# stm233/image-compression-for-machine

Measured on AMD Instinct MI355X. Metric: images/sec (256x256) cnn-hyperprior (WACNN) training step, higher is better.
Workload: dtype f32; 1 GPU; cnn (WACNN N=192 M=320) train step, lambda=0.0067 MSE, batch 16/GPU synthetic 256x256, Adam lr 1e-4 + aux Adam, clip 1.0; global_batch=16, parallelism=dp1

## Files before the change

image-compression-for-machine_amd/csrc/conv_igemm.hip:

```cpp
#include <cstdlib>
#include <vector>
#include "conv_common.h"

namespace icm {

template <int WCO, int WPX, int TCO, int TPX, int KS = 1>
__global__ __launch_bounds__(512, (TCO * TPX <= 3) ? 4 : 2) void conv_igemm_kernel(const ConvDesc d) {
  extern __shared__ __attribute__((aligned(16))) float smem[];
  static_assert(WCO * WPX * KS == 4, "4 MFMA waves per workgroup");
  constexpr int BCO_T = WCO * TCO;
  constexpr int TS = (TCO * TPX == 1) ? 3 : ((TCO * TPX == 2) ? 2 : 1);
  const int tid = threadIdx.x, lane = tid & 63, wave = tid >> 6;
  const bool loader = wave >= 4;
  const ConvPtrs P = d.g[blockIdx.y];
  const PatchGeom& pg = d.pg;

  int bid = xcd_block_id();
  const int cb = bid % d.ncb;
  int pt = bid / d.ncb;
  const int tx_i = pt % d.tiles_x;
  pt /= d.tiles_x;
  const int ty_i = pt % d.tiles_y;
  const int tn_i = pt / d.tiles_y;
  const int ox0 = tx_i << d.lgTW, oy0 = ty_i << d.lgTH, n0 = tn_i << d.lgTI;
  const int S_in = pg.S == 2 ? 2 : 1;
  const int iyb = oy0 * S_in + d.iy0, ixb = ox0 * S_in + d.ix0;
  const int bufsz = d.ckm * 8 * pg.CS;
  const int nchunks = (d.nchunks8 + d.ckm - 1) / d.ckm;

  if (loader) {
    const int lw = __builtin_amdgcn_readfirstlane(wave) - 4;
    PlaneMap pm;

    if (pg.dma) {
      plane_map_init(pm, pg, n0, iyb, ixb, lane);
      stage_planes_dma(P.x, pm, pg, 0, min(d.ckm, d.nchunks8) * 8, smem, lw, lane);
      asm volatile("s_waitcnt vmcnt(0)" ::: "memory");
      __syncthreads();
      for (int chunk = 0; chunk < nchunks; ++chunk) {
        if (chunk + 1 < nchunks) {
          const int c8 = (chunk + 1) * d.ckm;
          stage_planes_dma(P.x, pm, pg, c8 * 8, min(d.ckm, d.nchunks8 - c8) * 8, smem + ((chunk + 1) & 1) * bufsz, lw, lane);
          asm volatile("s_waitcnt vmcnt(0)" ::: "memory");
        }
        __syncthreads();
      }
      return;
    }
    if (pg.vec4) {
      plane_map_init_v4(pm, pg, n0, iyb, ixb, lane);
      stage_planes_v4<8>(P.x, pm, pg, 0, min(d.ckm, d.nchunks8) * 8, smem, lw);
      __syncthreads();
      for (int chunk = 0; chunk < nchunks; ++chunk) {
        if (chunk + 1 < nchunks) {
          const int c8 = (chunk + 1) * d.ckm;
          stage_planes_v4<8>(P.x, pm, pg, c8 * 8, min(d.ckm, d.nchunks8 - c8) * 8, smem + ((chunk + 1) & 1) * bufsz,
                             lw);
        }
        __syncthreads();
      }
      return;
    }
    plane_map_init(pm, pg, n0, iyb, ixb, lane);
    stage_planes<12>(P.x, pm, pg, 0, min(d.ckm, d.nchunks8) * 8, smem, lw);
    __syncthreads();
    for (int chunk = 0; chunk < nchunks; ++chunk) {
      if (chunk + 1 < nchunks) {
        const int c8 = (chunk + 1) * d.ckm;
        stage_planes<12>(P.x, pm, pg, c8 * 8, min(d.ckm, d.nchunks8 - c8) * 8, smem + ((chunk + 1) & 1) * bufsz, lw);
      }
      __syncthreads();
    }
    return;
  }

  const int wave_u = __builtin_amdgcn_readfirstlane(wave);
  const int wk = wave_u % KS, wsp = wave_u / KS;
  const int wco = wsp / WPX, wpx = wsp % WPX;
  const int h = lane >> 5, l31 = lane & 31;
  const int TWm = (1 << d.lgTW) - 1, THm = (1 << d.lgTH) - 1;
  const int rowmul = S_in * pg.PWrow;
  int boff[TPX];
// ... 57 lines not shown
        const int qq = (st * TS + u) * KS + wk;
        const int qc = min(qq, nq - 1);
        ok_n[u] = (qq < nq) ? 1.0f : 0.0f;
        const float* bp = cur + __builtin_amdgcn_readlane(step_lane, qc);
#pragma unroll
        for (int j = 0; j < 4; ++j)
#pragma unroll
          for (int tp = 0; tp < TPX; ++tp) bv_n[u][j][tp] = bp[boff[tp] + 2 * j * pg.CS];
      };
      auto half_step = [&](f32x4 (&aq)[TS][TCO], int st) {
        float bv[TS][4][TPX];
#pragma unroll
        for (int u = 0; u < TS; ++u)
#pragma unroll
          for (int j = 0; j < 4; ++j)
#pragma unroll
            for (int tp = 0; tp < TPX; ++tp) bv[u][j][tp] = bv_n[u][j][tp] * ok_n[u];
        const int stn = min(st + 1, nsteps2 - 1);
#pragma unroll
        for (int u = 0; u < TS; ++u) {
          const char* sp = wptr(chunk, st + 2, u);
#pragma unroll
          for (int a = 0; a < TCO; ++a) {
#pragma unroll
            for (int tp = 0; tp < TPX; ++tp)
#pragma unroll
              for (int j = 0; j < 4; ++j)
                acc[a][tp] = __builtin_amdgcn_mfma_f32_32x32x2f32(aq[u][a][j], bv[u][j][tp], acc[a][tp], 0, 0, 0);
            if (a == 0) bload(stn, u);
            aq[u][a] = *reinterpret_cast<const f32x4*>(sp + wl[a]);
            __builtin_amdgcn_sched_barrier(0);
          }
        }
      };
#pragma unroll
      for (int u = 0; u < TS; ++u) bload(0, u);
      for (int st = 0; st < nsteps2; st += 2) {
        half_step(aq0, st);
        half_step(aq1, st + 1);
      }
      __syncthreads();
    }
  }

  if constexpr (KS > 1) {
    static_assert(TCO == 1 && TPX == 1, "split-K configurations hold one tile per wave");
    float* red = smem + (wsp * (KS - 1)) * 1024;
    if (wk > 0) {
#pragma unroll
      for (int r = 0; r < 16; ++r) red[(wk - 1) * 1024 + r * 64 + lane] = acc[0][0][r];
    }
    __syncthreads();
    if (wk > 0) return;
#pragma unroll
    for (int k = 0; k < KS - 1; ++k)
#pragma unroll
      for (int r = 0; r < 16; ++r) acc[0][0][r] += red[k * 1024 + r * 64 + lane];
  }
  {
    int pn[TPX], poy[TPX], pox[TPX];
    bool pv[TPX];
#pragma unroll
    for (int tp = 0; tp < TPX; ++tp) {
      const int p = (wpx * TPX + tp) * 32 + l31;
      const int tx = p & TWm, ty = (p >> d.lgTW) & THm, ti = p >> (d.lgTW + d.lgTH);
      const int oyv = oy0 + ty, oxv = ox0 + tx;
      pn[tp] = n0 + ti;
      pv[tp] = (pn[tp] < d.pg.N) && (oyv < d.OHv) && (oxv < d.OWv);
      poy[tp] = oyv * d.out_sy + d.out_oy;
      pox[tp] = oxv * d.out_sx + d.out_ox;
    }
    epilogue_dispatch<TCO, TPX>(d, P, acc, cot0, h, pn, poy, pox, pv);
  }
}

struct PackDesc {
  const float* w;
  float* wp;
  int Co, Ci, KHW, src_out_major, ntaps, ncot, nchunks, nonneg;
  float bound, pedestal;
  int src_ld, src_off;
  int dst_ncot, dst_cot_off;
  int wino;
  short tapidx[ICM_MAX_TAPS];
};

#define ICM_PACK_LDS (8 * 32 * ICM_MAX_TAPS + 64)
__device__ __forceinline__ void pack_unit(const PackDesc& d, int cot, int chunk, float* lds) {
  const int KHW = d.KHW, tid = threadIdx.x;
  const int co0 = cot * 32, ci0 = chunk * 8;
  int rows, rlen, rstride;
  if (d.src_out_major) { rows = 32; rlen = 8 * KHW; } else { rows = 8; rlen = 32 * KHW; }
  rstride = rlen | 1;
  const int total = rows * rlen;
  for (int e0 = tid; e0 < total; e0 += 8 * (int)blockDim.x) {
    float v[8];
    int lo[8];
#pragma unroll
    for (int u = 0; u < 8; ++u) {
      const int e = e0 + u * (int)blockDim.x;
      v[u] = 0.0f;
      lo[u] = -1;
      if (e < total) {
        const int r = e / rlen, c = e - r * rlen;
        lo[u] = r * rstride + c;
        if (d.src_out_major) {
          const int co = co0 + r, ci = ci0 + c / KHW;
          if (co < d.Co && ci < d.Ci) v[u] = d.w[((long long)co * d.src_ld + d.src_off + ci0) * KHW + c];
        } else {
          const int ci = ci0 + r, co = co0 + c / KHW;
          if (ci < d.Ci && co < d.Co) v[u] = d.w[((long long)ci * d.src_ld + d.src_off + co0) * KHW + c];
        }
      }
    }
#pragma unroll
    for (int u = 0; u < 8; ++u) {
      if (lo[u] >= 0) {
        float x = v[u];
        if (d.nonneg) {
          x = fmaxf(x, d.bound);
          x = x * x - d.pedestal;
        }
        lds[lo[u]] = x;
      }
    }
  }
  __syncthreads();
  f32x4* out = reinterpret_cast<f32x4*>(d.wp);
  for (int e = tid; e < d.ntaps * 64; e += blockDim.x) {
    const int t = e >> 6, lane = e & 63;
    const int col = lane & 31, hh = lane >> 5, k = d.tapidx[t];
    f32x4 o;
#pragma unroll
    for (int j = 0; j < 4; ++j) {
      const int cil = 2 * j + hh;
      const float* gsrc = d.src_out_major ? lds + col * rstride + cil * KHW : lds + cil * rstride + col * KHW;
      float v;
      if (d.wino) {
        const int wa = t >> 2, wb = t & 3;
        float row[3];
#pragma unroll
        for (int p = 0; p < 3; ++p) {
          const float g0 = gsrc[d.wino == 2 ? (2 - p) * 3 + 2 : p * 3 + 0];
          const float g1 = gsrc[d.wino == 2 ? (2 - p) * 3 + 1 : p * 3 + 1];
          const float g2 = gsrc[d.wino == 2 ? (2 - p) * 3 + 0 : p * 3 + 2];
          row[p] = wb == 0 ? g0 : (wb == 3 ? g2 : (wb == 1 ? 0.5f * ((g0 + g2) + g1) : 0.5f * ((g0 + g2) - g1)));
        }
        v = wa == 0 ? row[0] : (wa == 3 ? row[2] : (wa == 1 ? 0.5f * ((row[0] + row[2]) + row[1]) : 0.5f * ((row[0] + row[2]) - row[1])));
      } else {
        v = gsrc[k];
      }
      const bool valid = (co0 + col < d.Co) && (ci0 + cil < d.Ci);
      o[j] = valid ? v : 0.0f;
    }
    out[((long long)(chunk * d.ntaps + t) * d.dst_ncot + d.dst_cot_off + cot) * 64 + lane] = o;
  }
  __syncthreads();
}

__global__ __launch_bounds__(256) void pack_weights_kernel(const PackDesc d) {
  __shared__ float lds[ICM_PACK_LDS];
  const int units = d.ncot * d.nchunks;
  for (int u = blockIdx.x; u < units; u += gridDim.x) pack_unit(d, u % d.ncot, u / d.ncot, lds);
}

#define ICM_PACK_NB 24
struct PackMulti {
  PackDesc g[ICM_PACK_NB];
};
__global__ __launch_bounds__(256) void pack_weights_multi_kernel(const PackMulti m) {
  __shared__ float lds[ICM_PACK_LDS];
  const PackDesc& d = m.g[blockIdx.y];
  const int units = d.ncot * d.nchunks;
  for (int u = blockIdx.x; u < units; u += gridDim.x) pack_unit(d, u % d.ncot, u / d.ncot, lds);
}

struct Tap {
  int kidx;
  int dy, dx;
};
struct ConvClass {
  int cy, cx;
  int iy0, ix0;
  int ey, ex;
  std::vector<Tap> taps;
};

static void axis_taps(int K, int s, int pad, int c, std::vector<int>& ks, std::vector<int>& dis) {
  for (int k = 0; k < K; ++k) {
    const int v = c + pad - k;
    if (((v % s) + s) % s != 0) continue;
    ks.push_back(k);
    dis.push_back(v >= 0 ? v / s : -((-v) / s));
  }
}

static std::vector<ConvClass> build_classes(int KH, int KW, int stride, int pad, int transposed) {
  std::vector<ConvClass> out;
  if (!transposed) {
    ConvClass c;
    c.cy = c.cx = 0;
    c.iy0 = c.ix0 = -pad;
    c.ey = KH;
    c.ex = KW;
    for (int kh = 0; kh < KH; ++kh)
      for (int kw = 0; kw < KW; ++kw) c.taps.push_back({kh * KW + kw, kh, kw});
    out.push_back(c);
    return out;
  }
  for (int cy = 0; cy < stride; ++cy)
    for (int cx = 0; cx < stride; ++cx) {
      std::vector<int> khs, dys, kws, dxs;
      axis_taps(KH, stride, pad, cy, khs, dys);
      axis_taps(KW, stride, pad, cx, kws, dxs);
      ConvClass c;
      c.cy = cy;
      c.cx = cx;
      int miny = 0, minx = 0, maxy = 0, maxx = 0;
      for (size_t i = 0; i < dys.size(); ++i) {
        miny = i ? std::min(miny, dys[i]) : dys[i];
        maxy = i ? std::max(maxy, dys[i]) : dys[i];
      }
      for (size_t i = 0; i < dxs.size(); ++i) {
        minx = i ? std::min(minx, dxs[i]) : dxs[i];
        maxx = i ? std::max(maxx, dxs[i]) : dxs[i];
      }
      c.iy0 = miny;
      c.ix0 = minx;
      c.ey = maxy - miny + 1;
      c.ex = maxx - minx + 1;
      for (size_t a = 0; a < khs.size(); ++a)
        for (size_t b = 0; b < kws.size(); ++b)
          c.taps.push_back({khs[a] * KW + kws[b], dys[a] - miny, dxs[b] - minx});
      out.push_back(c);
    }
  return out;
}

struct KernelCfg {
  int wco, wpx, tco, tpx;
  void (*fn)(const ConvDesc);
  int ks;
  double eff;
  int occ;
};
static const KernelCfg kCfgs[] = {
    {1, 4, 3, 2, conv_igemm_kernel<1, 4, 3, 2>, 1, 0.75, 1},
    {1, 4, 6, 1, conv_igemm_kernel<1, 4, 6, 1>, 1, 1.00, 1},
    {1, 4, 2, 2, conv_igemm_kernel<1, 4, 2, 2>, 1, 0.80, 1},
    {1, 4, 1, 2, conv_igemm_kernel<1, 4, 1, 2>, 1, 0.60, 2},
    {1, 4, 3, 1, conv_igemm_kernel<1, 4, 3, 1>, 1, 1.10, 2},
    {1, 4, 5, 1, conv_igemm_kernel<1, 4, 5, 1>, 1, 0.65, 1},
    {2, 2, 2, 1, conv_igemm_kernel<2, 2, 2, 1>, 1, 0.80, 2},
    {2, 2, 1, 1, conv_igemm_kernel<2, 2, 1, 1>, 1, 0.80, 2},
    {4, 1, 1, 1, conv_igemm_kernel<4, 1, 1, 1>, 1, 0.75, 2},
    {1, 4, 1, 1, conv_igemm_kernel<1, 4, 1, 1>, 1, 0.70, 2},
    {2, 1, 1, 1, conv_igemm_kernel<2, 1, 1, 1, 2>, 2, 0.70, 2},
// ... 173 lines not shown
  }
  if (p.family == kFamKs8) return launch_conv_ks8(d, p.row, p.nblk, ngroups, bg.lds_bytes, stream);
  const KernelCfg& c = kCfgs[p.row];
  if (bg.lds_bytes > 64 * 1024 && !ensure_max_lds(reinterpret_cast<const void*>(c.fn))) return ICM_ERR_LAUNCH;
  hipLaunchKernelGGL(c.fn, dim3((unsigned)p.nblk, ngroups, 1), dim3(p.block), bg.lds_bytes, stream, d);
  ICM_CHECK_LAUNCH();
  return ICM_OK;
}

static int validate(const icm_conv_args& a) {
  if (!a.x || !a.wp || !a.y) return ICM_ERR_ARG;
  if (a.N <= 0 || a.Cin <= 0 || a.Cout <= 0 || a.H <= 0 || a.W <= 0 || a.OH <= 0 || a.OW <= 0) return ICM_ERR_ARG;
  if (a.KH <= 0 || a.KW <= 0 || a.KH * a.KW > ICM_MAX_TAPS) return ICM_ERR_UNSUPPORTED;
  if (a.stride != 1 && a.stride != 2) return ICM_ERR_UNSUPPORTED;
  if (!a.transposed) {
    if (a.OH != (a.H + 2 * a.pad - a.KH) / a.stride + 1 || a.OW != (a.W + 2 * a.pad - a.KW) / a.stride + 1)
      return ICM_ERR_ARG;
  }
  if ((epi_reads_res(a.epi) && !a.res) || (epi_reads_aux(a.epi) && !a.aux) || (epi_reads_aux2(a.epi) && !a.aux2))
    return ICM_ERR_ARG;
  if (((long long)a.N * a.x_bs + 8LL * a.H * a.W) * 4 >= (1LL << 31)) return ICM_ERR_UNSUPPORTED;
  if (a.pixel_shuffle != 0 && a.pixel_shuffle != 2) return ICM_ERR_UNSUPPORTED;
  if (a.pixel_shuffle == 2 && (a.Cout % 4 != 0 || a.transposed)) return ICM_ERR_ARG;
  if (a.x_seg_len < 0 || (a.x_seg_len > 0 && (a.x_seg_gap < 0 || a.x_seg_len >= 65536))) return ICM_ERR_ARG;
  return ICM_OK;
}

static int check_group(const icm_conv_args* arr, int ngroups) {
  if (!arr || ngroups < 1 || ngroups > ICM_MAX_GROUPS) return ICM_ERR_ARG;
  for (int i = 0; i < ngroups; ++i) {
    int rc = validate(arr[i]);
    if (rc) return rc;
  }
  const icm_conv_args& a = arr[0];
  for (int i = 1; i < ngroups; ++i) {
    const icm_conv_args& b = arr[i];
    if (b.N != a.N || b.Cin != a.Cin || b.H != a.H || b.W != a.W || b.Cout != a.Cout || b.OH != a.OH || b.OW != a.OW ||
        b.KH != a.KH || b.KW != a.KW || b.stride != a.stride || b.pad != a.pad || b.transposed != a.transposed ||
        b.pro_act != a.pro_act || b.epi != a.epi || b.accum != a.accum || b.pixel_shuffle != a.pixel_shuffle ||
        b.x_bs != a.x_bs || b.y_bs != a.y_bs || b.x_seg_len != a.x_seg_len || b.x_seg_gap != a.x_seg_gap || b.algo != a.algo ||
        (b.res && b.res_bs != a.res_bs) || (b.aux && b.aux_bs != a.aux_bs) || (b.aux2 && b.aux2_bs != a.aux2_bs) ||
        (b.y2 && b.y2_bs != a.y2_bs) || (b.res != nullptr) != (a.res != nullptr) || (b.aux != nullptr) != (a.aux != nullptr) ||
        (b.aux2 != nullptr) != (a.aux2 != nullptr) || (b.y2 != nullptr) != (a.y2 != nullptr) ||
        (b.bias != nullptr) != (a.bias != nullptr) || (b.xv != nullptr) != (a.xv != nullptr))
      return ICM_ERR_ARG;
  }
  return (a.algo == ICM_ALGO_WINOGRAD || a.algo == ICM_ALGO_DIRECT) ? ICM_OK : ICM_ERR_ARG;
}

static long long class_packed_floats(int Cin, int ntaps, int ncot) { return (long long)cdiv(Cin, 8) * ntaps * ncot * 256; }

static bool x_aligned16(const icm_conv_args* arr, int ngroups) {
  bool ok = true;
  for (int gi = 0; gi < ngroups; ++gi) ok = ok && (reinterpret_cast<uintptr_t>(arr[gi].x) & 15) == 0;
  return ok;
}

static int conv_run_grouped(const icm_conv_args* arr, int ngroups, hipStream_t stream) {
  if (int rc = check_group(arr, ngroups)) return rc;
  const icm_conv_args& a = arr[0];
  if (a.algo == ICM_ALGO_WINOGRAD) return run_conv_wino(arr, ngroups, stream);
  const int S_in = a.transposed ? 1 : a.stride, out_s = a.transposed ? a.stride : 1;
  long long off = 0;
  for (const ConvClass& cls : build_classes(a.KH, a.KW, a.stride, a.pad, a.transposed)) {
    ConvPlan p;
    int rc = plan_class(a, ngroups, cls, S_in, out_s, x_aligned16(arr, ngroups), p);
    if (!rc) rc = launch_class(arr, ngroups, cls, off, S_in, out_s, p, stream);
    if (rc) return rc;
    off += class_packed_floats(a.Cin, (int)cls.taps.size(), cdiv(a.Cout, 32));
  }
  return ICM_OK;
}

static PackDesc make_pack_desc(const icm_pack_job& J, const ConvClass& cls, long long off) {
  const int ntaps = (int)cls.taps.size(), ncot = cdiv(J.Cout, 32);
  PackDesc d{};
  d.w = J.w;
  d.wp = J.wp + off;
  d.Co = J.Cout; d.Ci = J.Cin; d.KHW = J.KH * J.KW; d.src_out_major = J.src_out_major;
  d.ntaps = ntaps; d.ncot = ncot; d.nchunks = cdiv(J.Cin, 8); d.nonneg = J.nonneg;
  d.bound = J.bound; d.pedestal = J.pedestal;
  d.src_ld = J.src_ld > 0 ? J.src_ld : (J.src_out_major ? J.Cin : J.Cout); d.src_off = J.src_off;
  d.dst_ncot = J.dst_ncot > 0 ? J.dst_ncot : ncot; d.dst_cot_off = J.dst_cot_off; d.wino = J.wino;
  for (int t = 0; t < ntaps; ++t) d.tapidx[t] = (short)cls.taps[t].kidx;
  return d;
}

}

extern "C" {

int icm_conv_run(const icm_conv_args* a, void* stream) {
  return icm::conv_run_grouped(a, 1, (hipStream_t)stream);
}
int icm_conv_run_grouped(const icm_conv_args* a, int ngroups, void* stream) {
  return icm::conv_run_grouped(a, ngroups, (hipStream_t)stream);
}
int icm_conv2d_fwd(const icm_conv_args* a, void* stream) {
  if (!a || a->transposed) return ICM_ERR_ARG;
  return icm_conv_run(a, stream);
}
int icm_convT2d_dgrad(const icm_conv_args* a, void* stream) {
  if (!a || a->transposed) return ICM_ERR_ARG;
  return icm_conv_run(a, stream);
}
int icm_conv2d_dgrad(const icm_conv_args* a, void* stream) {
  if (!a || !a->transposed) return ICM_ERR_ARG;
  return icm_conv_run(a, stream);
}
int icm_convT2d_fwd(const icm_conv_args* a, void* stream) {
  if (!a || !a->transposed) return ICM_ERR_ARG;
  return icm_conv_run(a, stream);
}

int icm_conv_winograd_ok(const icm_conv_args* a) { return (a && icm::wino_supported(*a)) ? 1 : 0; }
int64_t icm_wino_transform_floats(const icm_conv_args* a) {
  return (a && icm::wino_supported(*a) && a->N > 0 && a->Cin > 0) ? (int64_t)icm::wino_transform_floats(*a) : -1;
}
int icm_wino_transform(const icm_conv_args* arr, int ngroups, void* stream) {
  if (!arr || ngroups < 1 || ngroups > ICM_MAX_GROUPS) return ICM_ERR_ARG;
  for (int i = 1; i < ngroups; ++i)
    if (arr[i].N != arr[0].N || arr[i].Cin != arr[0].Cin || arr[i].H != arr[0].H || arr[i].W != arr[0].W ||
        arr[i].x_bs != arr[0].x_bs || arr[i].pro_act != arr[0].pro_act || arr[i].x_seg_len != arr[0].x_seg_len ||
        arr[i].x_seg_gap != arr[0].x_seg_gap)
      return ICM_ERR_ARG;
  return icm::run_wino_transform(arr, ngroups, (hipStream_t)stream);
}

void icm_debug_force_conv_cfg(int idx) { icm::g_force_cfg = idx < 0 ? ICM_CONV_CFG_AUTO : idx; }
int icm_debug_forced_conv_cfg(void) { return icm::g_force_cfg; }
void icm_debug_force_conv1x1(int mode) { icm::g_force_1x1 = mode; }

int icm_debug_conv_plan(const icm_conv_args* arr, int ngroups, int cls, int64_t out[16]) {
  using namespace icm;
  std::fill(out, out + 16, 0);
  int rc = check_group(arr, ngroups);
  if (rc) return rc;
  const icm_conv_args& a = arr[0];
  if (a.algo == ICM_ALGO_WINOGRAD) {
    WinoPlan w{};
    if (cls != 0) return ICM_ERR_ARG;
    if ((rc = plan_conv_wino(a, ngroups, w))) return rc;
    const int64_t v[13] = {1, w.w8 ? kFamWino8 : kFamWino44, w.tco, w.g.lgTX, w.g.lgTY, w.g.lgTI, w.g.nsteps, w.ncb, w.nblk,
                           (int64_t)w.lds_bytes, 512, a.xv != nullptr, w.px_fast};
    std::copy(v, v + 13, out);
    return ICM_OK;
  }
  const std::vector<ConvClass> classes = build_classes(a.KH, a.KW, a.stride, a.pad, a.transposed);
  if (cls < 0 || cls >= (int)classes.size()) return ICM_ERR_ARG;
  long long off = 0;
  for (int i = 0; i < cls; ++i) off += class_packed_floats(a.Cin, (int)classes[i].taps.size(), cdiv(a.Cout, 32));
  ConvPlan p;
  rc = plan_class(a, ngroups, classes[cls], a.transposed ? 1 : a.stride, a.transposed ? a.stride : 1, x_aligned16(arr, ngroups), p);
  if (rc) return rc;
  const int64_t v[14] = {(int64_t)classes.size(), p.family, p.row, p.g.lgTW, p.g.lgTH, p.g.lgTI, p.g.ckm, p.ncb, p.nblk,
                         (int64_t)p.g.lds_bytes, p.block, p.vec4, p.dma, off};
  std::copy(v, v + 14, out);
  return ICM_OK;
}

int64_t icm_packed_weight_floats(int Cout, int Cin, int KH, int KW) {
  return icm::class_packed_floats(Cin, KH * KW, icm::cdiv(Cout, 32));
}

int icm_pack_weights(const float* w, float* wp, int Cout, int Cin, int KH, int KW, int src_out_major,
                     int transposed, int stride, int pad, int nonneg, float bound, float pedestal, void* stream) {
  using namespace icm;
  if (!w || !wp || Cout <= 0 || Cin <= 0 || KH * KW > ICM_MAX_TAPS || (stride != 1 && stride != 2)) return ICM_ERR_ARG;
  icm_pack_job J{};
  J.w = w; J.wp = wp; J.Cout = Cout; J.Cin = Cin; J.KH = KH; J.KW = KW; J.src_out_major = src_out_major; J.nonneg = nonneg;
  J.bound = bound; J.pedestal = pedestal;
  long long off = 0;
  for (const ConvClass& cls : build_classes(KH, KW, stride, pad, transposed)) {
    if (cls.taps.empty()) continue;
    const PackDesc d = make_pack_desc(J, cls, off);
    hipLaunchKernelGGL(pack_weights_kernel, dim3(std::min(d.nchunks * d.ncot, 2048)), dim3(256), 0, (hipStream_t)stream, d);
    ICM_CHECK_LAUNCH();
    off += class_packed_floats(Cin, d.ntaps, d.dst_ncot);
  }
  return ICM_OK;
}

int icm_pack_weights_batch(const icm_pack_job* jobs, int n, void* stream) {
  using namespace icm;
  if (!jobs || n < 1) return ICM_ERR_ARG;
  PackMulti m{};
  int nb = 0;
  auto flush = [&]() -> int {
    if (nb == 0) return ICM_OK;
    for (int i = nb; i < ICM_PACK_NB; ++i) m.g[i] = m.g[0];
    hipLaunchKernelGGL(pack_weights_multi_kernel, dim3(128, nb), dim3(256), 0, (hipStream_t)stream, m);
    ICM_CHECK_LAUNCH();
    nb = 0;
    return ICM_OK;
  };
  for (int k = 0; k < n; ++k) {
    const icm_pack_job& J = jobs[k];
    if (!J.w || !J.wp || J.Cout <= 0 || J.Cin <= 0 || J.KH * J.KW > ICM_MAX_TAPS || (J.stride != 1 && J.stride != 2))
      return ICM_ERR_ARG;
    std::vector<ConvClass> classes = build_classes(J.KH, J.KW, J.stride, J.pad, J.transposed);
    if (J.wino) {
      if (J.wino < 0 || J.wino > 2 || J.KH != 3 || J.KW != 3 || J.stride != 1 || J.pad != 1 || J.nonneg) return ICM_ERR_ARG;
      ConvClass wc;
      wc.cy = wc.cx = wc.iy0 = wc.ix0 = 0;
      wc.ey = wc.ex = 1;
      for (int t = 0; t < 16; ++t) wc.taps.push_back({0, 0, 0});
      classes.assign(1, wc);
    }
    const int ncot = cdiv(J.Cout, 32), inner = J.src_out_major ? J.Cin : J.Cout;
    if (J.src_off < 0 || J.src_off + inner > (J.src_ld > 0 ? J.src_ld : inner) || J.dst_cot_off < 0 ||
        J.dst_cot_off + ncot > (J.dst_ncot > 0 ? J.dst_ncot : ncot))
      return ICM_ERR_ARG;
    long long off = 0;
    for (const ConvClass& cls : classes) {
      if (cls.taps.empty()) continue;
      const PackDesc& d = m.g[nb] = make_pack_desc(J, cls, off);
      off += class_packed_floats(J.Cin, d.ntaps, d.dst_ncot);
      if (++nb == ICM_PACK_NB) {
        int rc = flush();
        if (rc) return rc;
      }
    }
  }
  return flush();
}

}
```

image-compression-for-machine_amd/csrc/conv_wino.hip:

```cpp
#include <cmath>
#include <cstdlib>
#include "conv_common.h"

namespace icm {

struct WinoDesc {
  ConvPtrs g[ICM_MAX_GROUPS];
  long long x_bs, y_bs, res_bs, aux_bs, y2_bs;
  int N, Cin, Cout, H, W;
  int lgTX, lgTY, lgTI, tiles_x, tiles_y, tiles_n;
  int ncot, nchunks8, ncb, nsteps;
  int epi, accum, act;
  int seg_len, seg_gap;
  FastDiv dseg;
  int dbg;
  int vpre;
  int px_fast, npx;
};

#define WINO_STEP_FLOATS (2 * 16 * 8 * 32)

template <int EPI>
__device__ __forceinline__ void wino_finish(const WinoDesc& d, const ConvPtrs& P, float v, int co, long long off, bool ok) {
  if (!ok) return;
  if (P.bias) v += P.bias[co];
  float side;
  v = epi_apply<EPI>(v, epi_reads_res(EPI) ? P.res[off] : 0.0f, epi_reads_aux(EPI) ? P.aux[off] : 0.0f, side);
  if constexpr (epi_writes_side(EPI))
    if (P.y2) P.y2[off] = side;
  if (d.accum) v += P.y[off];
  if constexpr (epi_may_gelu(EPI))
    if (P.y2) epi_materialise(v, P.y, P.y2, off, true);
  P.y[off] = v;
}

template <int TCO>
__global__ __launch_bounds__(512, 2) void conv_wino_kernel(const WinoDesc d) {
  extern __shared__ __attribute__((aligned(16))) float smem[];
  const int tid = threadIdx.x, lane = tid & 63;
  const int wave = __builtin_amdgcn_readfirstlane(tid >> 6);
  ConvPtrs P = d.g[blockIdx.y];
  int bid = xcd_block_id();
  const int cb = d.px_fast ? bid / d.npx : bid % d.ncb;
  int pt = d.px_fast ? bid % d.npx : bid / d.ncb;
  const int pblk = pt;
  const int bx = pt % d.tiles_x;
  pt /= d.tiles_x;
  const int by = pt % d.tiles_y;
  const int bn = pt / d.tiles_y;
  const int TXm = (1 << d.lgTX) - 1, TYm = (1 << d.lgTY) - 1;
  const int HW = d.H * d.W;

  if (wave >= 4 && d.vpre) {
    const int lw = wave - 4;
    const float* vsrc = P.x + (long long)pblk * (d.nsteps * 2) * 4096;
    auto dma = [&](int step, int buf) {
#pragma unroll
      for (int k = 0; k < 2; ++k)
#pragma unroll
        for (int rnd = 0; rnd < 4; ++rnd) {
          const int e = (rnd * 256 + lw * 64) * 4;
          __builtin_amdgcn_global_load_lds(vsrc + ((long long)(step * 2 + k) * 4096 + e + lane * 4),
                                           smem + buf * WINO_STEP_FLOATS + k * 4096 + e, 16, 0, 0);
        }
    };
    dma(0, 0);
    asm volatile("s_waitcnt vmcnt(0)" ::: "memory");
    __syncthreads();
    for (int s = 0; s < d.nsteps; ++s) {
      if (s + 1 < d.nsteps) dma(s + 1, (s + 1) & 1);
      asm volatile("s_waitcnt vmcnt(0)" ::: "memory");
      __syncthreads();
    }
  } else if (wave >= 4) {
    const int q = (wave - 4) * 64 + lane;
    const int ci_l = q >> 5, t = q & 31;
    const int tx = t & TXm, ty = (t >> d.lgTX) & TYm, ti = t >> (d.lgTX + d.lgTY);
    const int n = (bn << d.lgTI) + ti;
    const int oy = (((by << d.lgTY) + ty) << 1), ox = (((bx << d.lgTX) + tx) << 1);
    unsigned mask = 0;
#pragma unroll
    for (int dy = 0; dy < 4; ++dy)
#pragma unroll
      for (int dx = 0; dx < 4; ++dx) {
        const int iy = oy - 1 + dy, ix = ox - 1 + dx;
        if (n < d.N && (unsigned)iy < (unsigned)d.H && (unsigned)ix < (unsigned)d.W) mask |= 1u << (dy * 4 + dx);
      }
    const float* xbase = P.x + ((long long)n * d.x_bs + (long long)(oy - 1) * d.W + (ox - 1));
    const int act = d.act;
    auto load = [&](float (&r)[2][16], int step) {
#pragma unroll
      for (int k = 0; k < 2; ++k) {
        const int c = (step * 2 + k) * 8 + ci_l;
        const bool cok = c < d.Cin;
        const int cp = d.seg_len ? c + (int)fdiv((uint32_t)c, d.dseg) * d.seg_gap : c;
        const float* pc = xbase + (long long)cp * HW;
#pragma unroll
        for (int dy = 0; dy < 4; ++dy)
#pragma unroll
          for (int dx = 0; dx < 4; ++dx)
            r[k][dy * 4 + dx] = (cok && ((mask >> (dy * 4 + dx)) & 1u) && !(d.dbg & 1)) ? pc[dy * d.W + dx] : 0.0f;
      }
    };
    auto transform_store = [&](const float (&r)[2][16], int buf) {
      if (d.dbg & 8) return;
#pragma unroll
      for (int k = 0; k < 2; ++k) {
        float dd[16], u[16];
#pragma unroll
        for (int e = 0; e < 16; ++e) dd[e] = act ? apply_act(r[k][e], act) : r[k][e];
#pragma unroll
        for (int j = 0; j < 4; ++j) {
          u[0 * 4 + j] = dd[0 * 4 + j] - dd[2 * 4 + j];
          u[1 * 4 + j] = dd[1 * 4 + j] + dd[2 * 4 + j];
          u[2 * 4 + j] = dd[2 * 4 + j] - dd[1 * 4 + j];
          u[3 * 4 + j] = dd[1 * 4 + j] - dd[3 * 4 + j];
// ... 102 lines not shown
  if (P.y2) P.y2 += (long long)n * d.y2_bs;
  if (P.res) P.res += (long long)n * d.res_bs;
  if (P.aux) P.aux += (long long)n * d.aux_bs;
  auto finish_all = [&](auto epi_tag) {
    constexpr int EPI = decltype(epi_tag)::value;
#pragma unroll
    for (int a = 0; a < TCO; ++a) {
      const int cot = cot0 + a;
      if (cot >= d.ncot) continue;
#pragma unroll
      for (int i = 0; i < 2; ++i) {
        const int e = wave + 8 * i;
        const int co = cot * 32 + (e & 3) + 8 * (e >> 2) + 4 * h;
        float z[4][2];
#pragma unroll
        for (int rr = 0; rr < 4; ++rr)
#pragma unroll
          for (int cp = 0; cp < 2; ++cp) z[rr][cp] = zb[(((rr * 2 + cp) * TCO + a) * 16 + e) * 64 + lane];
        const bool cok = nok && co < d.Cout;
        const long long base = (long long)co * HW + (long long)oy * d.W + ox;
#pragma unroll
        for (int cp = 0; cp < 2; ++cp) {
          const float y0 = (z[0][cp] + z[1][cp]) + z[2][cp];
          const float y1 = (z[1][cp] - z[2][cp]) - z[3][cp];
          const bool xok = cok && ox + cp < d.W;
          wino_finish<EPI>(d, P, y0, co, base + cp, xok && oy < d.H);
          wino_finish<EPI>(d, P, y1, co, base + d.W + cp, xok && oy + 1 < d.H);
        }
      }
    }
  };
  if (d.dbg & 4) return;
  EpiWino::dispatch(d.epi, finish_all);
}


template <int TCO>
__global__ __launch_bounds__(512, 2) void conv_wino8_kernel(const WinoDesc d) {
  extern __shared__ __attribute__((aligned(16))) float smem[];
  const int tid = threadIdx.x, lane = tid & 63;
  const int wave = __builtin_amdgcn_readfirstlane(tid >> 6);
  ConvPtrs P = d.g[blockIdx.y];
  int bid = xcd_block_id();
  const int cb = d.px_fast ? bid / d.npx : bid % d.ncb;
  int pt = d.px_fast ? bid % d.npx : bid / d.ncb;
  const int pblk = pt;
  const int bx = pt % d.tiles_x;
  pt /= d.tiles_x;
  const int by = pt % d.tiles_y;
  const int bn = pt / d.tiles_y;
  const int TXm = (1 << d.lgTX) - 1, TYm = (1 << d.lgTY) - 1;
  const int HW = d.H * d.W;
  const int r = wave >> 1, ch = wave & 1;
  const int cot0 = cb * TCO;

  const float* vsrc = P.x + (long long)pblk * (d.nsteps * 2) * 4096;
  auto dma = [&](int step, int buf) {
#pragma unroll
    for (int i = 0; i < 4; ++i) {
      const int piece = wave + 8 * i;
      const int e = (piece >> 4) * 4096 + (piece & 15) * 256;
      __builtin_amdgcn_global_load_lds(vsrc + (long long)step * 8192 + e + lane * 4, smem + buf * WINO_STEP_FLOATS + e, 16, 0, 0);
    }
  };
  f32x16 acc[2][TCO];
#pragma unroll
  for (int c = 0; c < 2; ++c)
#pragma unroll
    for (int a = 0; a < TCO; ++a)
#pragma unroll
      for (int e = 0; e < 16; ++e) acc[c][a][e] = 0.0f;
  const char* wbase = reinterpret_cast<const char*>(P.wp);
  unsigned wl[TCO];
#pragma unroll
  for (int a = 0; a < TCO; ++a) wl[a] = (unsigned)(min(cot0 + a, d.ncot - 1) * 64 + lane) * 16u;
  const long long qstride = (long long)d.ncot * 64 * 16;
  const int nunits = d.nsteps * 4;
  const int lastq = d.nchunks8 * 16 - 1;
  const int xi0 = 4 * r + 2 * ch;
  auto wptr = [&](int g) -> const char* {
    const int qq = min((g >> 1) * 16 + xi0 + (g & 1), lastq);
    return wbase + qq * qstride;
  };
  dma(0, 0);
  f32x4 aq[4][TCO];
#pragma unroll
  for (int u = 0; u < 3; ++u)
#pragma unroll
    for (int a = 0; a < TCO; ++a) aq[u][a] = *reinterpret_cast<const f32x4*>(wptr(min(u, nunits - 1)) + wl[a]);
  const int boff = xi0 * 256 + lane;
  asm volatile("s_waitcnt vmcnt(0)" ::: "memory");
  __syncthreads();
  for (int s = 0; s < d.nsteps; ++s) {
    if (s + 1 < d.nsteps) dma(s + 1, (s + 1) & 1);
    const float* vb = smem + (s & 1) * WINO_STEP_FLOATS + boff;
    float bv[2][4];
#pragma unroll
    for (int j = 0; j < 4; ++j) bv[0][j] = vb[j * 64];
#pragma unroll
    for (int u = 0; u < 4; ++u) {
      const int g = s * 4 + u;
      if (u + 1 < 4) {
        const float* nb = vb + ((u + 1) >> 1) * (16 * 256) + ((u + 1) & 1) * 256;
#pragma unroll
        for (int j = 0; j < 4; ++j) bv[(u + 1) & 1][j] = nb[j * 64];
      }
      const char* sp = wptr(min(g + 3, nunits - 1));
#pragma unroll
      for (int a = 0; a < TCO; ++a) {
#pragma unroll
        for (int j = 0; j < 4; ++j)
          acc[u & 1][a] = __builtin_amdgcn_mfma_f32_32x32x2f32(aq[u][a][j], bv[u & 1][j], acc[u & 1][a], 0, 0, 0);
        aq[(u + 3) & 3][a] = *reinterpret_cast<const f32x4*>(sp + wl[a]);
      }
    }
    if constexpr (TCO == 4) asm volatile("s_waitcnt vmcnt(12)" ::: "memory");
    else if constexpr (TCO == 3) asm volatile("s_waitcnt vmcnt(9)" ::: "memory");
    else asm volatile("s_waitcnt vmcnt(6)" ::: "memory");
    asm volatile("s_waitcnt lgkmcnt(0)" ::: "memory");
    __builtin_amdgcn_s_barrier();
  }

  float* zb = smem;
  const int h = lane >> 5, l31 = lane & 31;
  const int tx = l31 & TXm, ty = (l31 >> d.lgTX) & TYm, ti = l31 >> (d.lgTX + d.lgTY);
  const int n = (bn << d.lgTI) + ti;
  const int oy = (((by << d.lgTY) + ty) << 1), ox = (((bx << d.lgTX) + tx) << 1);
  const bool nok = n < d.N;
  P.y += (long long)n * d.y_bs;
  if (P.y2) P.y2 += (long long)n * d.y2_bs;
  if (P.res) P.res += (long long)n * d.res_bs;
  if (P.aux) P.aux += (long long)n * d.aux_bs;
#pragma unroll
  for (int a0 = 0; a0 < TCO; a0 += 2) {
    __syncthreads();
#pragma unroll
    for (int al = 0; al < 2; ++al) {
      if (a0 + al >= TCO) break;
#pragma unroll
      for (int e = 0; e < 16; ++e) {
        const float m0 = acc[0][a0 + al][e], m1 = acc[1][a0 + al][e];
        const float p0 = ch == 0 ? m0 + m1 : m0;
        const float p1 = ch == 0 ? m1 : -m0 - m1;
        zb[((((al * 4 + r) * 2 + ch) * 2 + 0) * 16 + e) * 64 + lane] = p0;
        zb[((((al * 4 + r) * 2 + ch) * 2 + 1) * 16 + e) * 64 + lane] = p1;
      }
    }
    __syncthreads();
    auto finish_all = [&](auto epi_tag) {
      constexpr int EPI = decltype(epi_tag)::value;
#pragma unroll
      for (int al = 0; al < 2; ++al) {
        const int cot = cot0 + a0 + al;
        if (a0 + al >= TCO || cot >= d.ncot) continue;
#pragma unroll
        for (int i = 0; i < 2; ++i) {
          const int e = wave + 8 * i;
          const int co = cot * 32 + (e & 3) + 8 * (e >> 2) + 4 * h;
          float z[4][2];
#pragma unroll
          for (int rr = 0; rr < 4; ++rr)
#pragma unroll
            for (int cp = 0; cp < 2; ++cp)
              z[rr][cp] = zb[((((al * 4 + rr) * 2 + 0) * 2 + cp) * 16 + e) * 64 + lane] +
                          zb[((((al * 4 + rr) * 2 + 1) * 2 + cp) * 16 + e) * 64 + lane];
          const bool cok = nok && co < d.Cout;
          const long long base = (long long)co * HW + (long long)oy * d.W + ox;
#pragma unroll
          for (int cp = 0; cp < 2; ++cp) {
            const float y0 = (z[0][cp] + z[1][cp]) + z[2][cp];
            const float y1 = (z[1][cp] - z[2][cp]) - z[3][cp];
            const bool xok = cok && ox + cp < d.W;
            wino_finish<EPI>(d, P, y0, co, base + cp, xok && oy < d.H);
            wino_finish<EPI>(d, P, y1, co, base + d.W + cp, xok && oy + 1 < d.H);
          }
        }
      }
    };
    EpiWino::dispatch(d.epi, finish_all);
  }
}

bool wino_supported(const icm_conv_args& a);

struct WinoXfDesc {
  const float* x[ICM_MAX_GROUPS];
  float* v[ICM_MAX_GROUPS];
  long long x_bs;
  int N, Cin, H, W, lgTX, lgTY, lgTI, tiles_x, tiles_y, nchunks, act, seg_len, seg_gap;
  FastDiv dseg;
};
typedef float f32x4u __attribute__((ext_vector_type(4), aligned(4)));
template <bool VEC>
__global__ __launch_bounds__(256) void wino_input_transform_kernel(const WinoXfDesc d) {
  const float* x = d.x[blockIdx.y];
  float* v = d.v[blockIdx.y];
  const int chunk = blockIdx.x % d.nchunks;
  int pt = blockIdx.x / d.nchunks;
  const int pblk = pt;
  const int bx = pt % d.tiles_x;
  pt /= d.tiles_x;
  const int by = pt % d.tiles_y;
  const int bn = pt / d.tiles_y;
  const int q = threadIdx.x, ci_l = q >> 5, t = q & 31;
  const int TXm = (1 << d.lgTX) - 1, TYm = (1 << d.lgTY) - 1;
  const int tx = t & TXm, ty = (t >> d.lgTX) & TYm, ti = t >> (d.lgTX + d.lgTY);
  const int n = (bn << d.lgTI) + ti;
  const int oy = (((by << d.lgTY) + ty) << 1), ox = (((bx << d.lgTX) + tx) << 1);
  const int c = chunk * 8 + ci_l;
  const bool cok = c < d.Cin && n < d.N;
  const int cp = d.seg_len ? c + (int)fdiv((uint32_t)c, d.dseg) * d.seg_gap : c;
  const long long pbase = (long long)n * d.x_bs + (long long)cp * d.H * d.W + (long long)(oy - 1) * d.W + (ox - 1);
  float dd[16], u[16];
  if constexpr (VEC) {
    const bool tvalid = cok && ox < d.W;
    const bool left = ox == 0, right = ox == d.W - 2;
    f32x4u rv[4];
    bool rok[4];
#pragma unroll
    for (int dy = 0; dy < 4; ++dy) {
      rok[dy] = tvalid && (unsigned)(oy - 1 + dy) < (unsigned)d.H;
      const long long off = rok[dy] ? pbase + dy * d.W + (left ? 1 : (right ? -1 : 0)) : 0;
      rv[dy] = *reinterpret_cast<const f32x4u*>(x + off);
    }
#pragma unroll
    for (int dy = 0; dy < 4; ++dy) {
      const f32x4u w4 = rv[dy];
      float e[4];
      e[0] = left ? 0.0f : (right ? w4[1] : w4[0]);
      e[1] = left ? w4[0] : (right ? w4[2] : w4[1]);
      e[2] = left ? w4[1] : (right ? w4[3] : w4[2]);
      e[3] = left ? w4[2] : (right ? 0.0f : w4[3]);
#pragma unroll
      for (int dx = 0; dx < 4; ++dx) {
        const float val = rok[dy] ? e[dx] : 0.0f;
        dd[dy * 4 + dx] = d.act ? apply_act(val, d.act) : val;
      }
    }
  } else {
    const float* pc = x + pbase;
#pragma unroll
    for (int dy = 0; dy < 4; ++dy)
#pragma unroll
      for (int dx = 0; dx < 4; ++dx) {
        const int iy = oy - 1 + dy, ix = ox - 1 + dx;
        const float val = (cok && (unsigned)iy < (unsigned)d.H && (unsigned)ix < (unsigned)d.W) ? pc[dy * d.W + dx] : 0.0f;
        dd[dy * 4 + dx] = d.act ? apply_act(val, d.act) : val;
      }
  }
#pragma unroll
  for (int j = 0; j < 4; ++j) {
    u[0 * 4 + j] = dd[0 * 4 + j] - dd[2 * 4 + j];
    u[1 * 4 + j] = dd[1 * 4 + j] + dd[2 * 4 + j];
    u[2 * 4 + j] = dd[2 * 4 + j] - dd[1 * 4 + j];
    u[3 * 4 + j] = dd[1 * 4 + j] - dd[3 * 4 + j];
  }
  float* dst = v + ((long long)pblk * d.nchunks + chunk) * 4096 + ci_l * 32 + t;
#pragma unroll
  for (int i = 0; i < 4; ++i) {
    dst[(i * 4 + 0) * 256] = u[i * 4 + 0] - u[i * 4 + 2];
    dst[(i * 4 + 1) * 256] = u[i * 4 + 1] + u[i * 4 + 2];
    dst[(i * 4 + 2) * 256] = u[i * 4 + 2] - u[i * 4 + 1];
    dst[(i * 4 + 3) * 256] = u[i * 4 + 1] - u[i * 4 + 3];
// ... 127 lines not shown
```

Measured before the change: 386.9 images/s.

## Rework weight packing, deepen Winograd LDS prefetch, and vectorize Winograd epilogue stores

Weight packing now gives each block one work item, with a flat item index across the jobs of the multi-job kernel. The load phase is row-parallel and vectorized, 1x1 kernels group four Cin chunks per block, and each thread computes all 16 Winograd points at once instead of recomputing them per tap. The Winograd main loop prefetches two steps ahead for TCO!=3 and preloads B fragments across step boundaries, which drops an lgkmcnt wait. The epilogue writes adjacent output pairs as float2 when alignment allows. These target the per-step weight-pack overhead, LDS latency stalls and scalar stores, at the cost of more LDS buffers and added code complexity.

```diff
diff --git a/image-compression-for-machine_amd/csrc/conv_igemm.hip b/image-compression-for-machine_amd/csrc/conv_igemm.hip
--- a/image-compression-for-machine_amd/csrc/conv_igemm.hip
+++ b/image-compression-for-machine_amd/csrc/conv_igemm.hip
@@ -1,3 +1,4 @@
+#include <climits>
 #include <cstdlib>
 #include <vector>
 #include "conv_common.h"
@@ -221,97 +222,117 @@
   int src_ld, src_off;
   int dst_ncot, dst_cot_off;
   int wino;
+  int cg, ngroups;
+  int vec;
   short tapidx[ICM_MAX_TAPS];
 };
 
-#define ICM_PACK_LDS (8 * 32 * ICM_MAX_TAPS + 64)
-__device__ __forceinline__ void pack_unit(const PackDesc& d, int cot, int chunk, float* lds) {
+__host__ __device__ inline int pack_lds_floats(int cg, int KHW) { return 256 * cg * KHW + 32; }
+
+__device__ __forceinline__ float pack_nonneg(float x, float bound, float pedestal) {
+  x = fmaxf(x, bound);
+  x = x * x - pedestal;
+  return x;
+}
+
+__device__ __forceinline__ void pack_wino_points(const float* g, int wino, float (&u)[16]) {
+#pragma clang fp contract(off)
+  float row[3][4];
+#pragma unroll
+  for (int p = 0; p < 3; ++p) {
+    const float g0 = g[wino == 2 ? (2 - p) * 3 + 2 : p * 3 + 0];
+    const float g1 = g[wino == 2 ? (2 - p) * 3 + 1 : p * 3 + 1];
+    const float g2 = g[wino == 2 ? (2 - p) * 3 + 0 : p * 3 + 2];
+    row[p][0] = g0;
+    row[p][1] = 0.5f * ((g0 + g2) + g1);
+    row[p][2] = 0.5f * ((g0 + g2) - g1);
+    row[p][3] = g2;
+  }
+#pragma unroll
+  for (int b = 0; b < 4; ++b) {
+    u[0 * 4 + b] = row[0][b];
+    u[1 * 4 + b] = 0.5f * ((row[0][b] + row[2][b]) + row[1][b]);
+    u[2 * 4 + b] = 0.5f * ((row[0][b] + row[2][b]) - row[1][b]);
+    u[3 * 4 + b] = row[2][b];
+  }
+}
+
+__device__ __forceinline__ void pack_item(const PackDesc& d, int item, float* lds) {
   const int KHW = d.KHW, tid = threadIdx.x;
-  const int co0 = cot * 32, ci0 = chunk * 8;
-  int rows, rlen, rstride;
-  if (d.src_out_major) { rows = 32; rlen = 8 * KHW; } else { rows = 8; rlen = 32 * KHW; }
-  rstride = rlen | 1;
-  const int total = rows * rlen;
-  for (int e0 = tid; e0 < total; e0 += 8 * (int)blockDim.x) {
-    float v[8];
-    int lo[8];
-#pragma unroll
-    for (int u = 0; u < 8; ++u) {
-      const int e = e0 + u * (int)blockDim.x;
-      v[u] = 0.0f;
-      lo[u] = -1;
-      if (e < total) {
-        const int r = e / rlen, c = e - r * rlen;
-        lo[u] = r * rstride + c;
-        if (d.src_out_major) {
-          const int co = co0 + r, ci = ci0 + c / KHW;
-          if (co < d.Co && ci < d.Ci) v[u] = d.w[((long long)co * d.src_ld + d.src_off + ci0) * KHW + c];
-        } else {
-          const int ci = ci0 + r, co = co0 + c / KHW;
-          if (ci < d.Ci && co < d.Co) v[u] = d.w[((long long)ci * d.src_ld + d.src_off + co0) * KHW + c];
+  const int cot = item % d.ncot, grp = item / d.ncot;
+  const int co0 = cot * 32, chunk0 = grp * d.cg, ci0 = chunk0 * 8;
+  const int nch = min(d.cg, d.nchunks - chunk0);
+  const int som = d.src_out_major;
+  const int rows = som ? 32 : 8 * d.cg;
+  const int lgt = rows == 32 ? 3 : 5, tpr = 1 << lgt;
+  const int rlen = som ? 8 * d.cg * KHW : 32 * KHW, rstride = rlen | 1;
+  {
+    const int r = tid >> lgt, c0 = tid & (tpr - 1);
+    const int outer = (som ? co0 : ci0) + r, inner0 = som ? ci0 : co0;
+    const bool rok = outer < (som ? d.Co : d.Ci);
+    const int len = rok ? min(som ? 8 * nch : 32, (som ? d.Ci : d.Co) - inner0) * KHW : 0;
+    const float* src = d.w + ((long long)outer * d.src_ld + d.src_off + inner0) * KHW;
+    float* dst = lds + r * rstride;
+    const int n4 = d.vec ? len >> 2 : 0;
+    for (int b = c0; b < n4; b += 4 * tpr) {
+      f32x4 v[4];
+#pragma unroll
+      for (int u = 0; u < 4; ++u)
+        if (b + u * tpr < n4) v[u] = *reinterpret_cast<const f32x4*>(src + 4 * (b + u * tpr));
+#pragma unroll
+      for (int u = 0; u < 4; ++u)
+        if (b + u * tpr < n4) {
+#pragma unroll
+          for (int i = 0; i < 4; ++i) dst[4 * (b + u * tpr) + i] = d.nonneg ? pack_nonneg(v[u][i], d.bound, d.pedestal) : v[u][i];
         }
-      }
-    }
-#pragma unroll
-    for (int u = 0; u < 8; ++u) {
-      if (lo[u] >= 0) {
-        float x = v[u];
-        if (d.nonneg) {
-          x = fmaxf(x, d.bound);
-          x = x * x - d.pedestal;
-        }
-        lds[lo[u]] = x;
-      }
+    }
+    for (int b = 4 * n4 + c0; b < len; b += 8 * tpr) {
+      float v[8];
+#pragma unroll
+      for (int u = 0; u < 8; ++u)
+        if (b + u * tpr < len) v[u] = src[b + u * tpr];
+#pragma unroll
+      for (int u = 0; u < 8; ++u)
+        if (b + u * tpr < len) dst[b + u * tpr] = d.nonneg ? pack_nonneg(v[u], d.bound, d.pedestal) : v[u];
     }
   }
   __syncthreads();
-  f32x4* out = reinterpret_cast<f32x4*>(d.wp);
-  for (int e = tid; e < d.ntaps * 64; e += blockDim.x) {
-    const int t = e >> 6, lane = e & 63;
-    const int col = lane & 31, hh = lane >> 5, k = d.tapidx[t];
-    f32x4 o;
-#pragma unroll
-    for (int j = 0; j < 4; ++j) {
-      const int cil = 2 * j + hh;
-      const float* gsrc = d.src_out_major ? lds + col * rstride + cil * KHW : lds + cil * rstride + col * KHW;
-      float v;
-      if (d.wino) {
-        const int wa = t >> 2, wb = t & 3;
-        float row[3];
-#pragma unroll
-        for (int p = 0; p < 3; ++p) {
-          const float g0 = gsrc[d.wino == 2 ? (2 - p) * 3 + 2 : p * 3 + 0];
-          const float g1 = gsrc[d.wino == 2 ? (2 - p) * 3 + 1 : p * 3 + 1];
-          const float g2 = gsrc[d.wino == 2 ? (2 - p) * 3 + 0 : p * 3 + 2];
-          row[p] = wb == 0 ? g0 : (wb == 3 ? g2 : (wb == 1 ? 0.5f * ((g0 + g2) + g1) : 0.5f * ((g0 + g2) - g1)));
-        }
-        v = wa == 0 ? row[0] : (wa == 3 ? row[2] : (wa == 1 ? 0.5f * ((row[0] + row[2]) + row[1]) : 0.5f * ((row[0] + row[2]) - row[1])));
-      } else {
-        v = gsrc[k];
-      }
-      const bool valid = (co0 + col < d.Co) && (ci0 + cil < d.Ci);
-      o[j] = valid ? v : 0.0f;
-    }
-    out[((long long)(chunk * d.ntaps + t) * d.dst_ncot + d.dst_cot_off + cot) * 64 + lane] = o;
-  }
-  __syncthreads();
+  const int col = (tid >> 2) & 31, cil = 2 * (tid & 3) + (tid >> 7);
+  const long long tstride = (long long)d.dst_ncot * 256;
+  for (int cc = 0; cc < nch; ++cc) {
+    const int cl = cc * 8 + cil;
+    const float* gsrc = som ? lds + col * rstride + cl * KHW : lds + cl * rstride + col * KHW;
+    const bool valid = (co0 + col < d.Co) && (ci0 + cl < d.Ci);
+    float* out = d.wp + ((long long)(chunk0 + cc) * d.ntaps * d.dst_ncot + d.dst_cot_off + cot) * 256 + tid;
+    if (d.wino) {
+      float u[16];
+      pack_wino_points(gsrc, d.wino, u);
+#pragma unroll
+      for (int t = 0; t < 16; ++t) out[t * tstride] = valid ? u[t] : 0.0f;
+    } else {
+      for (int t = 0; t < d.ntaps; ++t) out[t * tstride] = valid ? gsrc[d.tapidx[t]] : 0.0f;
+    }
+  }
 }
 
 __global__ __launch_bounds__(256) void pack_weights_kernel(const PackDesc d) {
-  __shared__ float lds[ICM_PACK_LDS];
-  const int units = d.ncot * d.nchunks;
-  for (int u = blockIdx.x; u < units; u += gridDim.x) pack_unit(d, u % d.ncot, u / d.ncot, lds);
+  extern __shared__ float pack_lds[];
+  pack_item(d, blockIdx.x, pack_lds);
 }
 
 #define ICM_PACK_NB 24
 struct PackMulti {
   PackDesc g[ICM_PACK_NB];
+  int first[ICM_PACK_NB];
 };
+static_assert(sizeof(PackMulti) <= 4096, "kernel arguments are passed by value");
 __global__ __launch_bounds__(256) void pack_weights_multi_kernel(const PackMulti m) {
-  __shared__ float lds[ICM_PACK_LDS];
-  const PackDesc& d = m.g[blockIdx.y];
-  const int units = d.ncot * d.nchunks;
-  for (int u = blockIdx.x; u < units; u += gridDim.x) pack_unit(d, u % d.ncot, u / d.ncot, lds);
+  extern __shared__ float pack_lds[];
+  const int item = blockIdx.x;
+  int job = 0;
+#pragma unroll
+  for (int i = 1; i < ICM_PACK_NB; ++i) job += item >= m.first[i];
+  pack_item(m.g[job], item - m.first[job], pack_lds);
 }
 
 struct Tap {
@@ -651,9 +672,15 @@
   d.bound = J.bound; d.pedestal = J.pedestal;
   d.src_ld = J.src_ld > 0 ? J.src_ld : (J.src_out_major ? J.Cin : J.Cout); d.src_off = J.src_off;
   d.dst_ncot = J.dst_ncot > 0 ? J.dst_ncot : ncot; d.dst_cot_off = J.dst_cot_off; d.wino = J.wino;
+  d.cg = d.KHW == 1 ? 4 : 1;
+  d.ngroups = cdiv(d.nchunks, d.cg);
+  d.vec = (reinterpret_cast<uintptr_t>(J.w) & 15) == 0 && ((long long)d.src_ld * d.KHW) % 4 == 0 &&
+          ((long long)d.src_off * d.KHW) % 4 == 0;
   for (int t = 0; t < ntaps; ++t) d.tapidx[t] = (short)cls.taps[t].kidx;
   return d;
 }
+static int pack_items(const PackDesc& d) { return d.ncot * d.ngroups; }
+static size_t pack_lds_bytes(const PackDesc& d) { return sizeof(float) * pack_lds_floats(d.cg, d.KHW); }
 
 }
 
@@ -743,7 +770,7 @@
   for (const ConvClass& cls : build_classes(KH, KW, stride, pad, transposed)) {
     if (cls.taps.empty()) continue;
     const PackDesc d = make_pack_desc(J, cls, off);
-    hipLaunchKernelGGL(pack_weights_kernel, dim3(std::min(d.nchunks * d.ncot, 2048)), dim3(256), 0, (hipStream_t)stream, d);
+    hipLaunchKernelGGL(pack_weights_kernel, dim3(pack_items(d)), dim3(256), pack_lds_bytes(d), (hipStream_t)stream, d);
     ICM_CHECK_LAUNCH();
     off += class_packed_floats(Cin, d.ntaps, d.dst_ncot);
   }
@@ -757,8 +784,16 @@
   int nb = 0;
   auto flush = [&]() -> int {
     if (nb == 0) return ICM_OK;
-    for (int i = nb; i < ICM_PACK_NB; ++i) m.g[i] = m.g[0];
-    hipLaunchKernelGGL(pack_weights_multi_kernel, dim3(128, nb), dim3(256), 0, (hipStream_t)stream, m);
+    long long items = 0;
+    size_t lds = 0;
+    for (int i = 0; i < ICM_PACK_NB; ++i) {
+      m.first[i] = i < nb ? (int)items : INT_MAX;
+      if (i >= nb) continue;
+      items += pack_items(m.g[i]);
+      lds = std::max(lds, pack_lds_bytes(m.g[i]));
+    }
+    if (items > INT_MAX) return ICM_ERR_UNSUPPORTED;
+    hipLaunchKernelGGL(pack_weights_multi_kernel, dim3((unsigned)items), dim3(256), lds, (hipStream_t)stream, m);
     ICM_CHECK_LAUNCH();
     nb = 0;
     return ICM_OK;
diff --git a/image-compression-for-machine_amd/csrc/conv_wino.hip b/image-compression-for-machine_amd/csrc/conv_wino.hip
--- a/image-compression-for-machine_amd/csrc/conv_wino.hip
+++ b/image-compression-for-machine_amd/csrc/conv_wino.hip
@@ -32,6 +32,44 @@
   if constexpr (epi_may_gelu(EPI))
     if (P.y2) epi_materialise(v, P.y, P.y2, off, true);
   P.y[off] = v;
+}
+
+typedef float f32x2 __attribute__((ext_vector_type(2)));
+template <int EPI>
+__device__ __forceinline__ void wino_finish2(const WinoDesc& d, const ConvPtrs& P, float v0, float v1, int co, long long off,
+                                             bool ok) {
+  if (!ok) return;
+  if (P.bias) {
+    const float b = P.bias[co];
+    v0 += b;
+    v1 += b;
+  }
+  f32x2 rv = {0.0f, 0.0f}, av = {0.0f, 0.0f};
+  if constexpr (epi_reads_res(EPI)) rv = *reinterpret_cast<const f32x2*>(P.res + off);
+  if constexpr (epi_reads_aux(EPI)) av = *reinterpret_cast<const f32x2*>(P.aux + off);
+  float s0, s1;
+  v0 = epi_apply<EPI>(v0, rv[0], av[0], s0);
+  v1 = epi_apply<EPI>(v1, rv[1], av[1], s1);
+  if constexpr (epi_writes_side(EPI))
+    if (P.y2) *reinterpret_cast<f32x2*>(P.y2 + off) = f32x2{s0, s1};
+  if (d.accum) {
+    const f32x2 old = *reinterpret_cast<const f32x2*>(P.y + off);
+    v0 += old[0];
+    v1 += old[1];
+  }
+  if constexpr (epi_may_gelu(EPI))
+    if (P.y2) {
+      float g0 = v0, g1 = v1;
+      epi_materialise(g0, P.y, P.y, off, false);
+      epi_materialise(g1, P.y, P.y, off, false);
+      if (P.y2 == P.y) {
+        v0 = g0;
+        v1 = g1;
+      } else {
+        *reinterpret_cast<f32x2*>(P.y2 + off) = f32x2{g0, g1};
+      }
+    }
+  *reinterpret_cast<f32x2*>(P.y + off) = f32x2{v0, v1};
 }
 
 template <int TCO>
@@ -300,7 +338,9 @@
     const int qq = min((g >> 1) * 16 + xi0 + (g & 1), lastq);
     return wbase + qq * qstride;
   };
+  constexpr int AHEAD = TCO == 3 ? 1 : 2, SLOTM = 2 * AHEAD - 1;
   dma(0, 0);
+  if (AHEAD == 2 && d.nsteps > 1) dma(1, 1);
   f32x4 aq[4][TCO];
 #pragma unroll
   for (int u = 0; u < 3; ++u)
@@ -309,17 +349,24 @@
   const int boff = xi0 * 256 + lane;
   asm volatile("s_waitcnt vmcnt(0)" ::: "memory");
   __syncthreads();
+  float bv[2][4];
+  if constexpr (AHEAD == 2) {
+#pragma unroll
+    for (int j = 0; j < 4; ++j) bv[0][j] = (smem + boff)[j * 64];
+  }
   for (int s = 0; s < d.nsteps; ++s) {
-    if (s + 1 < d.nsteps) dma(s + 1, (s + 1) & 1);
-    const float* vb = smem + (s & 1) * WINO_STEP_FLOATS + boff;
-    float bv[2][4];
-#pragma unroll
-    for (int j = 0; j < 4; ++j) bv[0][j] = vb[j * 64];
+    if (s + AHEAD < d.nsteps) dma(s + AHEAD, (s + AHEAD) & SLOTM);
+    const float* vb = smem + (s & SLOTM) * WINO_STEP_FLOATS + boff;
+    if constexpr (AHEAD == 1) {
+#pragma unroll
+      for (int j = 0; j < 4; ++j) bv[0][j] = vb[j * 64];
+    }
 #pragma unroll
     for (int u = 0; u < 4; ++u) {
       const int g = s * 4 + u;
-      if (u + 1 < 4) {
-        const float* nb = vb + ((u + 1) >> 1) * (16 * 256) + ((u + 1) & 1) * 256;
+      if (u + 1 < 4 || AHEAD == 2) {
+        const float* nb = u + 1 < 4 ? vb + ((u + 1) >> 1) * (16 * 256) + ((u + 1) & 1) * 256
+                                    : smem + ((s + 1) & SLOTM) * WINO_STEP_FLOATS + boff;
 #pragma unroll
         for (int j = 0; j < 4; ++j) bv[(u + 1) & 1][j] = nb[j * 64];
       }
@@ -335,7 +382,7 @@
     if constexpr (TCO == 4) asm volatile("s_waitcnt vmcnt(12)" ::: "memory");
     else if constexpr (TCO == 3) asm volatile("s_waitcnt vmcnt(9)" ::: "memory");
     else asm volatile("s_waitcnt vmcnt(6)" ::: "memory");
-    asm volatile("s_waitcnt lgkmcnt(0)" ::: "memory");
+    if constexpr (AHEAD == 1) asm volatile("s_waitcnt lgkmcnt(0)" ::: "memory");
     __builtin_amdgcn_s_barrier();
   }
 
@@ -349,8 +396,12 @@
   if (P.y2) P.y2 += (long long)n * d.y2_bs;
   if (P.res) P.res += (long long)n * d.res_bs;
   if (P.aux) P.aux += (long long)n * d.aux_bs;
-#pragma unroll
-  for (int a0 = 0; a0 < TCO; a0 += 2) {
+  const ConvPtrs& P0 = d.g[blockIdx.y];
+  const bool pair = ((d.W | d.y_bs | d.y2_bs | d.res_bs | d.aux_bs) & 1) == 0 &&
+                    ((reinterpret_cast<uintptr_t>(P0.y) | reinterpret_cast<uintptr_t>(P0.y2) |
+                      reinterpret_cast<uintptr_t>(P0.res) | reinterpret_cast<uintptr_t>(P0.aux)) & 7) == 0;
+  auto pass = [&](auto a0_tag) {
+    constexpr int a0 = decltype(a0_tag)::value;
     __syncthreads();
 #pragma unroll
     for (int al = 0; al < 2; ++al) {
@@ -384,19 +435,31 @@
                           zb[((((al * 4 + rr) * 2 + 1) * 2 + cp) * 16 + e) * 64 + lane];
           const bool cok = nok && co < d.Cout;
           const long long base = (long long)co * HW + (long long)oy * d.W + ox;
+          float y0[2], y1[2];
 #pragma unroll
           for (int cp = 0; cp < 2; ++cp) {
-            const float y0 = (z[0][cp] + z[1][cp]) + z[2][cp];
-            const float y1 = (z[1][cp] - z[2][cp]) - z[3][cp];
-            const bool xok = cok && ox + cp < d.W;
-            wino_finish<EPI>(d, P, y0, co, base + cp, xok && oy < d.H);
-            wino_finish<EPI>(d, P, y1, co, base + d.W + cp, xok && oy + 1 < d.H);
+            y0[cp] = (z[0][cp] + z[1][cp]) + z[2][cp];
+            y1[cp] = (z[1][cp] - z[2][cp]) - z[3][cp];
+          }
+          if (pair) {
+            const bool xok = cok && ox < d.W;
+            wino_finish2<EPI>(d, P, y0[0], y0[1], co, base, xok && oy < d.H);
+            wino_finish2<EPI>(d, P, y1[0], y1[1], co, base + d.W, xok && oy + 1 < d.H);
+          } else {
+#pragma unroll
+            for (int cp = 0; cp < 2; ++cp) {
+              const bool xok = cok && ox + cp < d.W;
+              wino_finish<EPI>(d, P, y0[cp], co, base + cp, xok && oy < d.H);
+              wino_finish<EPI>(d, P, y1[cp], co, base + d.W + cp, xok && oy + 1 < d.H);
+            }
           }
         }
       }
     };
     EpiWino::dispatch(d.epi, finish_all);
-  }
+  };
+  pass(std::integral_constant<int, 0>{});
+  if constexpr (TCO > 2) pass(std::integral_constant<int, 2>{});
 }
 
 bool wino_supported(const icm_conv_args& a);
```

Result: faster. 398.7 images/s, median of 6 (+3.0%).
